# dayne-2stacks/Fingerprint-Matching-Code

Measured on AMD Instinct MI355X. Metric: graph-match pairs/sec @ n=256 kpts, batch=1024, 1 & 8 GPU, higher is better.
Workload: dtype bf16

## Files before the change

### fingerprint-matching-code_amd/_lib.py

```python
import ctypes
import os

_HERE = os.path.dirname(os.path.abspath(__file__))
LIB_PATH = os.environ.get("FPM_LIB_PATH") or os.path.join(_HERE, "libfpm_hip.so")

P = ctypes.c_void_p
I = ctypes.c_int
L = ctypes.c_long
F = ctypes.c_float

SIGNATURES = {
    "fpm_last_error": (ctypes.c_char_p, []),
    "fpm_version": (I, []),
    "fpm_device_sync": (I, []),
    "fpm_sinkhorn_log_fwd": (I, [P, L, L, L, P, L, L, L, P, P, I, I, I, I, F, I, P]),
    "fpm_sinkhorn_ws_bytes": (L, [I, I, I]),
    "fpm_sinkhorn_log_fwd_ws": (I, [P, L, L, L, P, L, L, L, P, P, I, I, I, I, F, I, P, L, P]),
    "fpm_soft_topk_fwd": (I, [P, L, L, P, P, P, I, I, I, I, F, P, L, L, P, P, L, L, P]),
    "fpm_topk_select": (I, [P, L, L, P, L, P, I, I, I, P, L, L, P, L, L, P]),
    "fpm_greedy_perm": (I, [P, L, I, P, I, I, I, P, L, L, P]),
    "fpm_gemm": (I, [I, P, L, L, P, P, L, L, I, I, I, I, I, P, P, P, L, L, P, P, P]),
    "fpm_cast_bf16": (I, [P, P, L, P]),
    "fpm_global_weights": (I, [P, L, P, L, I, I, I, P, L, P]),
    "fpm_coef_tanh": (I, [P, L, P, P, I, I, I, P, L, P]),
    "fpm_split_bf16x3": (I, [P, L, L, I, I, P, L, P]),
    "fpm_set_tuning": (I, [ctypes.c_char_p, I]),
    "fpm_spline_plan_bytes": (L, [L, L]),
    "fpm_spline_plan": (I, [P, P, P, L, L, I, P, L, P]),
    "fpm_spline_plan_graphs": (I, [P, P, P, L, L, I, L, P, L, P]),
    "fpm_spline_plan_csr": (I, [P, L, L, ctypes.POINTER(P), ctypes.POINTER(P)]),
    "fpm_spline_plan_edges": (I, [P, L, L, ctypes.POINTER(P), ctypes.POINTER(P), ctypes.POINTER(P)]),
    "fpm_spline_plan_multi": (I, [P, I, I, I, P, P]),
    "fpm_spline_plan_job_bytes": (I, []),
    "fpm_spline_y_bytes": (L, [I, L, L]),
    "fpm_spline_conv_fwd": (I, [I, P, P, L, L, I, P, P, P, P, L, I, P, P, P, P, P]),
    "fpm_spline_conv_fwd_argmax": (I, [I, P, P, L, L, I, P, P, P, P, L, I, P, P, P, P, P, P]),
    "fpm_edge_diff": (I, [P, P, P, L, I, P, P]),
    "fpm_rows_bcast_scale": (I, [I, P, L, I, P, P, P, I, P]),
    "fpm_rows_gather_scale": (I, [I, P, P, P, I, I, I, P, P, P, I, P]),
    "fpm_rank_topk": (I, [P, L, I, I, I, P, P, P]),
    "fpm_rank_select_ws_bytes": (L, [I]),
    "fpm_rank_select": (I, [P, L, I, I, I, P, P, P, L, P]),
    "fpm_group_scores": (I, [P, L, I, I, P, L, P, L, I, I, P, P, P]),
    "fpm_coarse_score_wide_ws_bytes": (L, [I]),
    "fpm_coarse_score_stream_ws_bytes": (L, [I, I, I]),
    "fpm_rows_fetch": (I, [P, L, P, P, I, I, I, P, L, P, P]),
    "fpm_rows_pack": (I, [P, L, P, I, I, P, P, P, L, P]),
    "fpm_edge_diff_padded":(I, [P, P, P, P, P, P, L, I, P, P]),
    "fpm_kron_gnn_layer_fwd": (I, [P, I, I, I, I, P, P, P, P, P, P, P, P, P, P, P, P]),
    "fpm_kron_gnn_layer_fwd_ord": (I, [P, I, I, I, I, P, P, P, P, P, P, P, P, P, P, P, P, P]),
    "fpm_gnn_param_count": (I, [I]),
    "fpm_node_classifier": (I, [P, I, I, I, P, P, P, P, P]),
    "fpm_crossset_attn_fwd": (I, [I, P, L, L, I, I, I, P, P, I, P, P, P, P, P, P, P]),
    "fpm_instnorm": (I, [I, P, P, I, I, I, P, P, P, P, F, P, P, I, P, P]),
    "fpm_afau_head": (I, [P, P, I, I, P, P, P, P, P, P, P, P, P, P]),
    "fpm_afau_head_bwd": (I, [P, P, I, I, P, P, P, P, P, P, P, P, P, P, P, P, P]),
    "fpm_instnorm_bwd": (I, [P, P, I, I, I, P, P, P, P, F, P, P, P, I, P, P, P]),
    "fpm_afau_attn_bwd": (I, [P, L, L, I, I, I, P, P, I, P, P, P, P, P, P, P, P, P, P]),
    "fpm_rows_sum": (I, [P, I, L, P, I, P, I, P]),
    "fpm_transpose": (I, [P, L, I, L, P, L, P]),
    "fpm_elementwise": (I, [P, P, L, I, P]),
    "fpm_outer_sum_parts": (L, [I, L]),
    "fpm_outer_sum": (I, [P, L, L, I, P, L, L, I, I, I, L, P, P]),
    "fpm_bn_ws_floats": (L, [I, I]),
    "fpm_bn_relu_train_fwd": (I, [P, I, I, L, P, P, F, F, P, P, P, P, P, P]),
    "fpm_bn_relu_train_bwd": (I, [P, P, I, I, L, P, P, P, P, P, P, P]),
    "fpm_match_cls_ws_floats": (L, [I, I, I]),
    "fpm_match_cls_fwd": (I, [I, P, P, I, I, I, P, P, P, P, P, P, P, P, P, P, P, P, P, P]),
    "fpm_match_cls_train_ws_floats": (L, [I, I, I, I]),
    "fpm_match_cls_train_fwd": (I, [P, P, I, I, I] + [P] * 14 + [ctypes.c_float, ctypes.c_float, P, P, P, P]),
    "fpm_match_cls_train_bwd": (I, [P, P, I, I, I] + [P] * 21 + [P]),
    "fpm_gemm_norm_max": (I, [P, L, P, L, I, I, I, P, P, L, P, P, ctypes.c_float, I, P, P]),
    "fpm_gemm_norm_out": (I, [P, L, P, L, I, I, I, P, P, P, ctypes.c_float, I, P, L, P, L, P]),
    "fpm_affinity_ws_floats": (L, [I, I, I]),
    "fpm_perm_loss_fwd": (I, [P, L, L, P, L, L, P, P, I, I, I, P, P, P, P]),
    "fpm_perm_loss_bwd": (I, [P, L, L, P, L, L, P, P, I, I, I, P, P, P, P]),
    "fpm_affinity_fwd": (I, [P, L, P, L, P, I, P, P, I, I, I, I, P, P, I, P, L, P, L, P]),
    "fpm_gemm_x3out": (I, [P, L, P, L, I, I, I, I, P, P, P, ctypes.c_float, I, P, L, P, L, I, P]),
    "fpm_lsa_batch_host": (I, [P, L, L, P, P, I, I, P, I]),
    "fpm_lsa_submit": (L, [P, L, L, P, P, I, I, P, I]),
    "fpm_lsa_wait": (I, [L, I, ctypes.POINTER(ctypes.c_double)]),
    "fpm_lsa_batch_device": (I, [P, L, L, P, P, I, I, I, P, P, P]),
    "fpm_csr_dot_csc_to_dense": (I, [I, P, P, P, P, P, P, L, L, L, P, P]),
    "fpm_dense_dot_csc_to_dense": (I, [I, P, P, P, P, L, L, L, L, P, P]),
    "fpm_csr_dot_diag_to_csr": (I, [I, P, P, P, P, L, L, L, P, P]),
    "fpm_bilinear_diag": (I, [I, P, P, P, P, L, P, P, P, L, L, P, P]),
    "fpm_csr_dot_csc_to_csr_host": (L, [I, P, P, P, P, P, P, L, L, L, P, L, P, P]),
    "fpm_csr_dot_diag_to_csr_host": (I, [I, P, P, P, P, L, L, L, P]),
    "fpm_bilinear_diag_host": (I, [I, P, P, P, P, L, P, P, P, L, L, P]),
    "fpm_gconv_ws_floats": (L, [I, I, I]),
    "fpm_gconv_fwd": (I, [P, P, I, I, I, I, P, P, I, P, P, P]),
    "fpm_graph_words": (I, [I]),
    "fpm_graph_build": (I, [P, P, I, I, I, ctypes.c_double, P, P, P, P, P]),
    "fpm_graph_edges": (I, [P, P, P, P, I, I, ctypes.c_double, P, P, P, P, P, P, I, P]),
    "fpm_kron_pattern": (I, [P, P, L, P, P, L, I, I, I, I, P, P, P]),
    "fpm_feature_align_ws_floats": (L, [P, P]),
    "fpm_feature_align_fwd": (I, [P, P, P, P, P, P, P, P, I, F, F, P, P, L, P, P]),
    "fpm_feature_align_bwd": (I, [P, P, P, P, P, P, P, P, I, F, F, P, P, L, P, P, P, P, P, P]),
    "fpm_sinkhorn_bwd_ws_floats": (L, [I, I, I, I]),
    "fpm_sinkhorn_log_bwd": (I, [P, L, L, L, P, L, L, L, P, P, P, I, I, I, I, F, I, P, L, P]),
    "fpm_soft_topk_bwd_ws_floats": (L, [I, I, I]),
    "fpm_soft_topk_bwd": (I, [P, L, L, P, P, P, P, I, I, I, F, P, L, L, P, P, L, P, P]),
    "fpm_spline_plan_rows": (I, [P, L, L, ctypes.POINTER(P), ctypes.POINTER(P)]),
    "fpm_spline_conv_bwd_data": (I, [I, P, L, L, I, P, P, P, I, P, P, P, P, P, P, I, P]),
# ... 56 lines not shown
```

### fingerprint-matching-code_amd/csrc/gemm.hip

```cpp
#include "gemm_phase.h"
#include <cstdlib>
#include <cstring>

namespace fpm {
int& gemm_bn256_min();
}
int& gemm_store_sc1_flag();

extern "C" int fpm_gemm(int dtype, const void* A, long lda, long sA, const int* a_rows, const void* B, long ldb,
                        long sB, int M, int N, int K, int batch, int epi, const float* bias, float* Cf, void* Ct,
                        long ldc, long sC, const int* n1, const int* n2, void* stream) {
    using namespace fpm;
    FPM_CHECK_ARG(dtype == 0 || dtype == 1, "gemm: dtype must be 0 (f32) or 1 (bf16)");
    FPM_CHECK_ARG(M >= 0 && N > 0 && K > 0 && batch >= 0, "gemm: bad sizes M=%d N=%d K=%d", M, N, K);
    FPM_CHECK_ARG(K % (dtype ? 8 : 4) == 0, "gemm: K=%d must be a multiple of %d", K, dtype ? 8 : 4);
    FPM_CHECK_ARG(lda % (dtype ? 8 : 4) == 0 && ldb % (dtype ? 8 : 4) == 0, "gemm: lda/ldb must keep rows 16-B aligned");
    FPM_CHECK_ARG((epi != EPI_AFFINITY && epi != EPI_HALF_AFFINITY) || (n1 && n2),
                  "gemm: affinity epilogues need n1/n2");
    FPM_CHECK_ARG(epi >= EPI_STORE && epi <= EPI_HALF_AFFINITY, "gemm: bad epilogue %d", epi);
    if (M == 0 || batch == 0) return 0;
    GemmParams p = {};
    p.A = A; p.lda = lda; p.sA = sA; p.a_rows = a_rows;
    p.B = B; p.ldb = ldb; p.sB = sB; p.sB_seg = 0;
    p.row_scale = nullptr;
// ... 154 lines not shown
    else hipLaunchKernelGGL((gemm_big_kernel<128, EPI_STORE, true>), grid, dim3(G2_THREADS), 0, st, p);
    return check_launch("fpm_gemm_x3out");
}

namespace {
__global__ __launch_bounds__(256) void rows_scale_kernel(const float* __restrict__ X, long ldx, int nmax, int d,
                                                         const float* __restrict__ coef, float* __restrict__ Xc) {
    const long r = blockIdx.x;
    const int b = (int)(r / nmax);
    for (int k = threadIdx.x; k < d; k += 256) Xc[r * d + k] = X[r * ldx + k] * coef[(long)b * d + k];
}
}

extern "C" long fpm_affinity_ws_floats(int B, int n1max, int d) { return (long)B * d + (long)B * n1max * d; }

extern "C" int fpm_affinity_fwd(const float* X1, long ld1, const float* X2, long ld2, const float* w, int kw,
                                const float* A_w, const float* A_b, int B, int n1max, int n2max, int d, const int* n1,
                                const int* n2, int epi, float* K, long ldk, float* ws, long ws_floats, void* stream) {
    using namespace fpm;
    FPM_CHECK_ARG(epi == 0 || epi == 1, "affinity_fwd: epi must be 0 (vertex) or 1 (edge)");
    FPM_CHECK_ARG(B >= 0 && n1max > 0 && n2max > 0 && d > 0 && d % 4 == 0 && kw > 0 && kw % 4 == 0,
                  "affinity_fwd: bad sizes");
    FPM_CHECK_ARG(ld1 >= d && ld2 >= d && ld2 % 4 == 0 && ldk >= n2max, "affinity_fwd: bad strides");
    FPM_CHECK_ARG(ws && ws_floats >= fpm_affinity_ws_floats(B, n1max, d), "affinity_fwd: workspace too small");
    FPM_CHECK_ARG(n1 && n2 && K && X1 && X2 && w && A_w, "affinity_fwd: null operand");
    if (B == 0) return 0;
    float* coef = ws;
    float* X1c = ws + (long)B * d;
    if (fpm_gemm(0, w, kw, 0, nullptr, A_w, kw, 0, B, d, kw, 1, EPI_TANH, A_b, coef, nullptr, d, 0, nullptr, nullptr,
                 stream))
        return 1;
    hipLaunchKernelGGL(rows_scale_kernel, dim3((unsigned)((long)B * n1max)), dim3(256), 0, (hipStream_t)stream, X1,
                       ld1, n1max, d, coef, X1c);
    if (check_launch("fpm_affinity_fwd")) return 1;
    return fpm_gemm(0, X1c, d, (long)n1max * d, nullptr, X2, ld2, (long)n2max * ld2, n1max, n2max, d, B,
                    epi == 0 ? EPI_AFFINITY : EPI_HALF_AFFINITY, nullptr, K, nullptr, ldk, (long)n1max * ldk, n2, n1,
                    stream);
}

int& plan_graph_flag();
int& combine_npb_flag();
int& sinkhorn_bwd_reg_flag();
int& sinkhorn_fast_flag();
int& sinkhorn_lform_flag();
int& soft_topk_fast_flag();
int& afau_attn_v_flag();
int& gnn_store_sc1_flag();
int& combine_store_sc1_flag();
int& gemm_store_sc1_flag();
int& combine_lds_kb_flag();
int& gnn_mlp_off_flag();
int& outer_sum_vec_flag();
int& gnn_sweeps_flag();
int& scatter_f32_rows_flag();
int& scatter_batch_flag();
int& afau_head_split_flag();

extern "C" int fpm_set_tuning(const char* key, int value) {
    int* f = nullptr;
    if (key && !strcmp(key, "gemm_phase")) f = &fpm::gemm_phase_flag();
    else if (key && !strcmp(key, "gemm_walk")) f = &fpm::gemm_walk_flag();
    else if (key && !strcmp(key, "gemm_bn256_min")) f = &fpm::gemm_bn256_min();
    else if (key && !strcmp(key, "plan_graph")) f = &plan_graph_flag();
    else if (key && !strcmp(key, "combine_npb")) f = &combine_npb_flag();
    else if (key && !strcmp(key, "sinkhorn_bwd_reg")) f = &sinkhorn_bwd_reg_flag();
    else if (key && !strcmp(key, "sinkhorn_fast")) f = &sinkhorn_fast_flag();
    else if (key && !strcmp(key, "sinkhorn_lform")) f = &sinkhorn_lform_flag();
    else if (key && !strcmp(key, "topk_fast")) f = &soft_topk_fast_flag();
    else if (key && !strcmp(key, "afau_attn_v")) f = &afau_attn_v_flag();
    else if (key && !strcmp(key, "gnn_store_sc1")) f = &gnn_store_sc1_flag();
    else if (key && !strcmp(key, "combine_store_sc1")) f = &combine_store_sc1_flag();
    else if (key && !strcmp(key, "gemm_store_sc1")) f = &gemm_store_sc1_flag();
    else if (key && !strcmp(key, "combine_lds_kb")) f = &combine_lds_kb_flag();
    else if (key && !strcmp(key, "gnn_mlp_off")) f = &gnn_mlp_off_flag();
    else if (key && !strcmp(key, "outer_sum_vec")) f = &outer_sum_vec_flag();
    else if (key && !strcmp(key, "gnn_sweeps")) f = &gnn_sweeps_flag();
    else if (key && !strcmp(key, "scatter_f32_rows")) f = &scatter_f32_rows_flag();
    else if (key && !strcmp(key, "scatter_batch")) f = &scatter_batch_flag();
    else if (key && !strcmp(key, "afau_head_split")) f = &afau_head_split_flag();
    if (!f) {
        fpm::set_error("fpm_set_tuning: unknown key '%s'", key ? key : "(null)");
        return -1;
    }
    if (f == &gnn_mlp_off_flag() && value != 0) {
        const char* e = getenv("FPM_TIMING_PROBES");
        if (!e || strcmp(e, "1") != 0) {
            fpm::set_error("fpm_set_tuning: '%s' is a timing probe with wrong results; set FPM_TIMING_PROBES=1 "
                           "to allow it", key);
            return -1;
        }
    }
    const int prev = *f;
    *f = value;
    return prev;
}

namespace {
__global__ void cast_bf16_kernel(const float* __restrict__ x, bf16_t* __restrict__ y, long n) {
    long i = (long)blockIdx.x * blockDim.x + threadIdx.x;
    long stride = (long)gridDim.x * blockDim.x;
    for (; i < n; i += stride) y[i] = fpm::f2bf(x[i]);
}

__global__ __launch_bounds__(256) void cast_bf16_v8_kernel(const float4* __restrict__ x, uint4* __restrict__ y, long n8) {
    const long i = (long)blockIdx.x * blockDim.x + threadIdx.x;
    if (i >= n8) return;
    const float4 a = x[2 * i], b = x[2 * i + 1];
    uint4 o;
    o.x = (uint32_t)fpm::f2bf(a.x) | ((uint32_t)fpm::f2bf(a.y) << 16);
    o.y = (uint32_t)fpm::f2bf(a.z) | ((uint32_t)fpm::f2bf(a.w) << 16);
    o.z = (uint32_t)fpm::f2bf(b.x) | ((uint32_t)fpm::f2bf(b.y) << 16);
    o.w = (uint32_t)fpm::f2bf(b.z) | ((uint32_t)fpm::f2bf(b.w) << 16);
    y[i] = o;
}
}

extern "C" int fpm_cast_bf16(const float* x, void* y, long n, void* stream) {
    if (n <= 0) return 0;
    if (n % 8 == 0 && ((uintptr_t)x & 15) == 0 && ((uintptr_t)y & 15) == 0) {
        const long n8 = n / 8;
        hipLaunchKernelGGL(cast_bf16_v8_kernel, dim3((unsigned)((n8 + 255) / 256)), dim3(256), 0, (hipStream_t)stream,
                           (const float4*)x, (uint4*)y, n8);
        return fpm::check_launch("fpm_cast_bf16");
    }
    long blocks = (n + 255) / 256;
    if (blocks > 65536) blocks = 65536;
    hipLaunchKernelGGL(cast_bf16_kernel, dim3(blocks), dim3(256), 0, (hipStream_t)stream, x, (bf16_t*)y, n);
    return fpm::check_launch("fpm_cast_bf16");
}
// ... 122 lines not shown
```

### fingerprint-matching-code_amd/csrc/gnn.hip

```cpp
#include "fpm_common.h"
#include <cstdlib>

namespace {

__device__ __forceinline__ bool pair_block(int n2max, int B, int& b, int& d) {
    const int x = blockIdx.x & 7, k = blockIdx.x >> 3;
    b = (k / n2max) * 8 + x;
    d = k % n2max;
    return b < B;
}

inline unsigned pair_grid(int n2max, int B) { return (unsigned)(((B + 7) / 8) * 8 * n2max); }

template <int C>
struct GnnPack {
    static constexpr int Wl = 0, bl = Wl + 16 * C, Wr = bl + 16, W1 = Wr + 16 * C, b1 = W1 + 16 * C, W2 = b1 + 16,
                         b2 = W2 + 256, wc = b2 + 16, bc = wc + 16, total = bc + 1;
};

typedef float f2_t __attribute__((ext_vector_type(2)));

__device__ __forceinline__ void pk_fma_bcast(f2_t& acc, f2_t w, f2_t v, bool hi) {
    if (hi) asm("v_pk_fma_f32 %0, %1, %2, %0 op_sel:[0,1,0] op_sel_hi:[1,1,1]" : "+v"(acc) : "s"(w), "v"(v));
    else asm("v_pk_fma_f32 %0, %1, %2, %0 op_sel_hi:[1,0,1]" : "+v"(acc) : "s"(w), "v"(v));
}

template <int C, int TS, int SPOL = 0, bool MLP = true>
__device__ __forceinline__ void gnn_point(const float* Tg, __amdgpu_buffer_rsrc_t xr, int N4, long N, int n1max,
                                          int b, int d, int i, int nn2, const int* __restrict__ ptr1,
                                          const int* __restrict__ nbr1, int n1b, int n2b, const float* __restrict__ W,
                                          float* __restrict__ Xo, float* __restrict__ zbuf, float* __restrict__ vpart,
                                          const float* __restrict__ cls_w) {
    using P = GnnPack<C>;
    const long p = (long)d * n1max + i;
    const __amdgpu_buffer_rsrc_t orr = __builtin_amdgcn_make_buffer_rsrc((void*)(Xo + (long)b * 17 * N), (short)0,
                                                                         (int)(17 * N * 4), 0x00020000);
    auto store_o = [&](int o, float v) {
        __builtin_amdgcn_raw_buffer_store_b32(__float_as_uint(v), orr, (int)p * 4, o * N4, SPOL);
    };
    const int beg = ptr1[(long)b * n1max + i], end = ptr1[(long)b * n1max + i + 1];
    const bool self = p < (long)n1b * n2b;
    float x[C], agg[C];
#pragma unroll
    for (int c = 0; c < C; ++c) {
        x[c] = __uint_as_float(__builtin_amdgcn_raw_buffer_load_b32(xr, (int)p * 4, c * N4, 0));
        agg[c] = 0.f;
    }
    for (int e = beg; e < end; ++e) {
        const float* Ta = Tg + nbr1[e] * TS;
        if constexpr (C == 17) {
            static_assert(TS % 4 == 0, "16-B aligned node rows");
#pragma unroll
            for (int q = 0; q < 4; ++q) {
// ... 110 lines not shown
                load_row(nbr2[k], va);
#pragma unroll
                for (int c = 0; c < C; ++c) acc[c] += va[c];
            }
        } else {
            constexpr int GS = (C + NSW - 1) / NSW;
#pragma unroll
            for (int g0 = 0; g0 < C; g0 += GS) {
                int k = beg2;
                for (; k + 3 < end2; k += 4) {
                    float v[4][GS];
#pragma unroll
                    for (int u = 0; u < 4; ++u) {
                        const int r = nbr2[k + u];
#pragma unroll
                        for (int c = 0; c < GS; ++c)
                            if (g0 + c < C)
                                v[u][c] = __uint_as_float(__builtin_amdgcn_raw_buffer_load_b32(xr, (r * n1max + i) * 4,
                                                                                                (g0 + c) * N4, 0));
                    }
#pragma unroll
                    for (int u = 0; u < 4; ++u)
#pragma unroll
                        for (int c = 0; c < GS; ++c)
                            if (g0 + c < C) acc[g0 + c] += v[u][c];
                }
                for (; k < end2; ++k) {
                    const int r = nbr2[k];
#pragma unroll
                    for (int c = 0; c < GS; ++c)
                        if (g0 + c < C)
                            acc[g0 + c] += __uint_as_float(__builtin_amdgcn_raw_buffer_load_b32(xr, (r * n1max + i) * 4,
                                                                                                 (g0 + c) * N4, 0));
                }
            }
        }
        float* Ti = T + i * TS;
        if constexpr (C == 17) {
#pragma unroll
            for (int q = 0; q < 4; ++q)
                *(float4*)(Ti + 4 * q) = make_float4(acc[4 * q], acc[4 * q + 1], acc[4 * q + 2], acc[4 * q + 3]);
            Ti[16] = acc[16];
        } else {
            Ti[0] = acc[0];
        }
    }
    __syncthreads();
    if (i >= n1max) return;
    gnn_point<C, TS, SPOL, MLP>(T, xr, N4, N, n1max, b, d, i, end2 - beg2, ptr1, nbr1, n1[b], n2[b], W, Xo, zbuf,
                                vpart, cls_w);
    (void)NSW;
}

__global__ __launch_bounds__(256) void node_classifier_t_kernel(const float* __restrict__ X, int n1max, int n2max,
                                                                const float* __restrict__ w,
                                                                const float* __restrict__ bias,
                                                                const float* __restrict__ vpart,
                                                                float* __restrict__ s) {
    __shared__ float tile[64][65];
    const int b = blockIdx.z, d0 = blockIdx.y * 64, i0 = blockIdx.x * 64;
    const int tx = threadIdx.x & 63, ty = threadIdx.x >> 6;
    const long N = (long)n1max * n2max;
    const float* Xb = X + (long)b * 17 * N;
    const int i = i0 + tx;
#pragma unroll 4
    for (int r = 0; r < 16; ++r) {
        const int d = d0 + ty + 4 * r;
        if (d < n2max && i < n1max) {
            const long p = (long)d * n1max + i;
            float acc;
            if (vpart) {
                acc = fmaf(w[16], Xb[16L * N + p], vpart[(long)b * N + p]);
            } else {
                acc = 0.f;
#pragma unroll
                for (int c = 0; c < 17; ++c) acc += w[c] * Xb[(long)c * N + p];
            }
            tile[tx][ty + 4 * r] = acc + bias[0];
        }
    }
    __syncthreads();
    const int d = d0 + tx;
#pragma unroll 4
    for (int r = 0; r < 16; ++r) {
        const int ii = i0 + ty + 4 * r;
        if (ii < n1max && d < n2max) s[(long)b * N + (long)ii * n2max + d] = tile[ty + 4 * r][tx];
    }
}

}

int& gnn_sweeps_flag() {
    static int v = [] {
        const char* e = getenv("FPM_GNN_SWEEPS");
        return e ? atoi(e) : 1;
    }();
    return v;
}

int& gnn_store_sc1_flag() {
    static int v = [] {
        const char* e = getenv("FPM_GNN_SC1");
        return e ? atoi(e) : 0;
    }();
    return v;
}

int& gnn_mlp_off_flag() {
    static int v = 0;
    return v;
}

extern "C" int fpm_kron_gnn_layer_fwd_ord(const float* X, int C, int B, int n1max, int n2max, const int* ptr1,
                                          const int* nbr1, const int* ptr2, const int* nbr2, const int* n1,
                                          const int* n2, const float* params, float* Xout, float* zbuf,
                                          float* vpart, const float* cls_w, const int* ord2, void* stream) {
    FPM_CHECK_ARG(C == 1 || C == 17, "gnn_layer: C must be 1 or 17 (got %d)", C);
    FPM_CHECK_ARG(!vpart || cls_w, "gnn_layer: vpart needs cls_w");
    if (B == 0) return 0;
    FPM_CHECK_ARG(n1max >= 1 && n1max <= 1024, "gnn_layer: n1max must be in [1, 1024]");
    FPM_CHECK_ARG((long)17 * n1max * n2max * 4 < (1L << 31), "gnn_layer: a pair's state must be < 2 GiB");
    const size_t sh = (size_t)(C == 1 ? 1 : 20) * n1max * 4;
    const int threads = (n1max + 63) / 64 * 64;
    void (*k)(const float*, int, int, const int*, const int*, const int*, const int*, const int*, const int*,
              const float*, float*, float*, float*, const float*, int, const int*) =
        (C == 17 && gnn_sweeps_flag() == 2 && !gnn_mlp_off_flag() && !gnn_store_sc1_flag()) ? gnn_layer_kernel<17, 0, true, 2>
        : (C == 17 && gnn_sweeps_flag() == 3 && !gnn_mlp_off_flag() && !gnn_store_sc1_flag()) ? gnn_layer_kernel<17, 0, true, 3>
        : gnn_mlp_off_flag() ? (C == 1 ? gnn_layer_kernel<1, 0, false> : gnn_layer_kernel<17, 0, false>)
        : gnn_store_sc1_flag() ? (C == 1 ? gnn_layer_kernel<1, 16> : gnn_layer_kernel<17, 16>)
                               : (C == 1 ? gnn_layer_kernel<1> : gnn_layer_kernel<17>);
    if (sh > 65536) (void)hipFuncSetAttribute((const void*)k, hipFuncAttributeMaxDynamicSharedMemorySize, (int)sh);
    hipLaunchKernelGGL(k, dim3(pair_grid(n2max, B)), dim3(threads), sh, (hipStream_t)stream, X, n1max, n2max, ptr1,
                       nbr1, ptr2, nbr2, n1, n2, params, Xout, zbuf, vpart, cls_w, B, ord2);
    return fpm::check_launch("fpm_kron_gnn_layer_fwd");
}

extern "C" int fpm_kron_gnn_layer_fwd(const float* X, int C, int B, int n1max, int n2max, const int* ptr1,
                                      const int* nbr1, const int* ptr2, const int* nbr2, const int* n1,
                                      const int* n2, const float* params, float* Xout, float* zbuf,
                                      float* vpart, const float* cls_w, void* stream) {
    return fpm_kron_gnn_layer_fwd_ord(X, C, B, n1max, n2max, ptr1, nbr1, ptr2, nbr2, n1, n2, params, Xout, zbuf,
                                      vpart, cls_w, nullptr, stream);
}

extern "C" int fpm_gnn_param_count(int C) { return C == 1 ? GnnPack<1>::total : GnnPack<17>::total; }

extern "C" int fpm_node_classifier(const float* X, int B, int n1max, int n2max, const float* w, const float* bias,
                                   const float* vpart, float* s, void* stream) {
    if (B == 0) return 0;
    FPM_CHECK_ARG(B <= 65535, "node_classifier: B must be <= 65535");
    const dim3 grid((unsigned)((n1max + 63) / 64), (unsigned)((n2max + 63) / 64), (unsigned)B);
    hipLaunchKernelGGL(node_classifier_t_kernel, grid, dim3(256), 0, (hipStream_t)stream, X, n1max, n2max, w, bias,
                       vpart, s);
    return fpm::check_launch("fpm_node_classifier");
}

namespace {
__global__ __launch_bounds__(1024) void kron_agg_kernel(const float* __restrict__ X, int C, int n1max, int n2max,
                                                        const int* __restrict__ tptr1, const int* __restrict__ tnbr1,
                                                        const int* __restrict__ tptr2, const int* __restrict__ tnbr2,
                                                        const int* __restrict__ q1, const int* __restrict__ q2,
                                                        const int* __restrict__ n1, const int* __restrict__ n2,
                                                        int adj_flags, float* __restrict__ out, int B) {
    extern __shared__ float T[];
    int d, b;
    if (!pair_block(n2max, B, b, d)) return;
    const int adj = adj_flags & 1;
    const bool accum = (adj_flags & 2) != 0;
    const int i = threadIdx.x;
    const long N = (long)n1max * n2max;
    const float* Xb = X + (long)b * C * N;
    const long nb1 = (long)b * n1max, nb2 = (long)b * n2max;
    const long nn = (long)n1[b] * n2[b];
    auto den = [&](int dd, int ii) -> float {
        const int g1 = q1[nb1 + ii + 1] - q1[nb1 + ii];
        const int g2 = q2[nb2 + dd + 1] - q2[nb2 + dd];
        return (float)(g1 * g2 + (((long)dd * n1max + ii) < nn ? 1 : 0));
    };
    auto xval = [&](int c, int dd, int ii) -> float {
        const float x = Xb[(long)c * N + (long)dd * n1max + ii];
        if (!adj) return x;
        const float dn = den(dd, ii);
        return dn > 0.f ? x / dn : 0.f;
// ... 205 lines not shown
```

### fingerprint-matching-code_amd/ops.py

```python
import ctypes

import torch

from . import _lib

F32, BF16 = 0, 1
EPI_STORE, EPI_RELU, EPI_TANH, EPI_AFFINITY, EPI_HALF_AFFINITY = 0, 1, 2, 3, 4
EPI_NORM_OUT = 6


def _p(t):
    return ctypes.c_void_p(0 if t is None else t.data_ptr())


def _stream(t=None):
    dev = t.device if t is not None else torch.device("cuda")
    return ctypes.c_void_p(torch.cuda.current_stream(dev).cuda_stream)


def _dev(*ts):
    for t in ts:
        if t is not None and not t.is_cuda:
            raise _lib.FpmError("fpm op called with a CPU tensor: the HIP path has no CPU fallback")

# ... 780 lines not shown
            raise _lib.FpmError("%s: qidx value outside [0, %d)" % (op, Q))
        ng, nq = oh[gh + 1] - oh[gh], qoh[qh + 1] - qoh[qh]
        nqmax, ngmax = int(nq.max()), int(ng.max())
        for what, n in (("probe", nq), ("selected entry", ng)):
            if int(n.max()) > nmax or int(n.min()) < 1:
                raise _lib.FpmError("%s: a %s of %d keypoints; the %s coarse pass takes 1 to %s = %d"
                                    % (op, what, int(n.max()) if int(n.max()) > nmax else int(n.min()), kernel, bound,
                                       nmax))
    iters, tau = _check_iters_tau(op, iters, tau)
    if not y.is_cuda:
        dtype = _host_dtype(op, dtype)
        res = torch.empty(B, dtype=dtype)
        for b in range(B):
            q = int(qh[b])
            res[b:b + 1] = _coarse_score_host(y, oh, gh[b:b + 1], yq[int(qoh[q]):int(qoh[q + 1])], coef[b:b + 1], iters,
                                              tau, dtype)
        return _coarse_out(op, y, B, out, dtype, res)
    out = _coarse_out(op, y, B, out, dtype)
    if B:
        _coarse_call(kernel, True, y, (_p(y), _p(row_off), _p(gidx), G, B, _p(yq), _p(qrow_off), _p(qidx), Q, _p(coef),
                                       iters, tau, _p(out)), B, nqmax, ngmax)
    return out


def edge_diff(x, src, dst):
    _dev(x, src, dst)
    E, D = src.numel(), x.shape[-1]
    out = torch.empty(E, D, device=x.device, dtype=torch.float32)
    _lib.call("fpm_edge_diff", _p(x), _p(src), _p(dst), E, D, _p(out), _stream(x))
    return out


def edge_diff_padded(x, src, dst, pair, row, nrows, cscale=None):
    _dev(x, src, dst, pair, row)
    E, D = src.numel(), x.shape[-1]
    out = torch.zeros(nrows, D, device=x.device, dtype=torch.float32)
    _lib.call("fpm_edge_diff_padded", _p(x), _p(src), _p(dst), _p(pair), _p(row), _p(cscale), E, D, _p(out),
              _stream(x))
    return out


def gnn_layer(X, C, B, n1max, n2max, csr1, csr2, n1, n2, params, Xout, zbuf, vpart=None, cls_w=None, ord2=None):
    _dev(X, n1, n2, params, Xout, zbuf, vpart, cls_w, ord2)
    _shape(X, (B, C, n2max, n1max), "gnn_layer X")
    _shape(Xout, (B, 17, n2max, n1max), "gnn_layer Xout")
    _shape(zbuf, (B, n2max, n1max), "gnn_layer zbuf")
    _shape(vpart, (B, n2max, n1max), "gnn_layer vpart")
    _shape(ord2, (B, n2max), "gnn_layer ord2")
    _lib.call("fpm_kron_gnn_layer_fwd_ord", _p(X), C, B, n1max, n2max, ctypes.c_void_p(csr1[0]),
              ctypes.c_void_p(csr1[1]), ctypes.c_void_p(csr2[0]), ctypes.c_void_p(csr2[1]), _p(n1), _p(n2),
              _p(params), _p(Xout), _p(zbuf), _p(vpart), _p(cls_w), _p(ord2), _stream(X))


def node_classifier(X, B, n1max, n2max, w, b, out, vpart=None):
    _dev(X, w, b, out, vpart)
    _shape(X, (B, 17, n2max, n1max), "node_classifier X")
    _shape(out, (B, n1max, n2max), "node_classifier out")
    _shape(vpart, (B, n2max, n1max), "node_classifier vpart")
    _lib.call("fpm_node_classifier", _p(X), B, n1max, n2max, _p(w), _p(b), _p(vpart), _p(out), _stream(X))


def crossset_attn(cost, n2, Wv, mix1w, mix1b, mix2w, mix2b, out, split=False, stats=None):
    _dev(cost, n2, Wv, out)
    B, n1max, n2max = cost.shape
    _shape(out, (B * n1max, 768 if split else 256), "crossset_attn out")
    if split and out.dtype != torch.bfloat16:
        raise _lib.FpmError("crossset_attn: split rows are bf16")
    _shape(stats, (B * n1max, 16, 2), "crossset_attn stats")
    if n2max > 1 and cost.stride(2) != 1:
        raise _lib.FpmError("crossset_attn: cost rows must be contiguous (inner stride %d)" % cost.stride(2))
    _lib.call("fpm_crossset_attn_fwd", 2 if split else _code(out), _p(cost), cost.stride(0), cost.stride(1), B, n1max, n2max,
              _p(n2), _p(Wv), Wv.shape[1], _p(mix1w), _p(mix1b), _p(mix2w), _p(mix2b), _p(out), _p(stats),
              _stream(cost))


def instnorm(in1, B, P, Cn, w, b, in2=None, nvalid=None, onehot_bias=None, out_f=None, out_t=None, gmax=None,
             eps=1e-5, ldt=0):
    code = _code(out_t) if out_t is not None else F32
    ref = in1 if in1 is not None else w
    _lib.call("fpm_instnorm", code, _p(in1), _p(in2), B, P, Cn, _p(nvalid), _p(onehot_bias), _p(w), _p(b),
              float(eps), _p(out_f), _p(out_t), int(ldt), _p(gmax), _stream(ref))


def gemm_norm_max(A, Bw, M, N, K, lda, ldb, bias, res, nw, nb, gmax, P=256, eps=1e-5):
    _dev(A, Bw, res, gmax)
    _lib.call("fpm_gemm_norm_max", _p(A), int(lda), _p(Bw), int(ldb), int(M), int(N), int(K), _p(bias), _p(res),
              int(res.stride(0)), _p(nw), _p(nb), float(eps), int(P), _p(gmax), _stream(A))
    return gmax


def gemm_norm_out(A, Bw, M, N, K, lda, ldb, bias, nw, nb, out_f, out_t=None, ldt=0, P=256, eps=1e-5):
    _dev(A, Bw, out_f)
    _lib.call("fpm_gemm_norm_out", _p(A), int(lda), _p(Bw), int(ldb), int(M), int(N), int(K), _p(bias), _p(nw),
              _p(nb), float(eps), int(P), _p(out_f), int(out_f.stride(0)), _p(out_t),
              int(ldt or (out_t.stride(0) if out_t is not None else 0)), _stream(A))
    return out_f


def affinity(X1, X2, w, A_w, A_b, n1, n2, half=False, out=None):
    _dev(X1, X2, w, A_w, A_b, n1, n2)
    for t in (X1, X2, w, A_w, A_b):
        if t.dtype != torch.float32:
            raise _lib.FpmError("affinity: float32 operands expected")
    B, n1max, d = X1.shape
    n2max = X2.shape[1]
    kw = w.shape[1]
# ... 537 lines not shown
```

### include/fpm.h

```cpp
#ifndef FPM_H_
#define FPM_H_

#ifdef __cplusplus
extern "C" {
#endif

const char* fpm_last_error(void);
int fpm_version(void);
int fpm_device_sync(void);

int fpm_sinkhorn_log_fwd(const float* s, long s_sb, long s_si, long s_sj, float* out, long o_sb, long o_si,
                         long o_sj, const int* n1, const int* n2, int B, int n1max, int n2max, int iters,
                         float tau, int dummy_row, void* stream);
long fpm_sinkhorn_ws_bytes(int B, int n1max, int n2max);
int fpm_sinkhorn_log_fwd_ws(const float* s, long s_sb, long s_si, long s_sj, float* out, long o_sb, long o_si,
                            long o_sj, const int* n1, const int* n2, int B, int n1max, int n2max, int iters,
                            float tau, int dummy_row, void* ws, long ws_bytes, void* stream);

int fpm_soft_topk_fwd(const float* ss, long s_sb, long s_ld, const int* n1, const int* n2, const float* k, int B,
                      int n1max, int n2max, int iters, float tau, float* out, long o_sb, long o_ld, int* steps_out,
                      float* out2, long o2_sb, long o2_ld, void* stream);

int fpm_topk_select(const float* ds, long d_sb, long d_ld, const int* assign, long a_sb, const float* k, int B,
                    int n1max, int n2max, float* perm, long p_sb, long p_ld, float* lsa_out, long l_sb, long l_ld,
// ... 21 lines not shown
                  long ldo, void* stream);
long fpm_affinity_ws_floats(int B, int n1max, int d);
int fpm_affinity_fwd(const float* X1, long ld1, const float* X2, long ld2, const float* w, int kw, const float* A_w,
                     const float* A_b, int B, int n1max, int n2max, int d, const int* n1, const int* n2, int epi,
                     float* K, long ldk, float* ws, long ws_floats, void* stream);

int fpm_perm_loss_fwd(const float* ds, long d_sb, long d_ld, const float* gt, long g_sb, long g_ld, const int* n1,
                      const int* n2, int B, int n1max, int n2max, float* ws, int* bad, float* out, void* stream);
int fpm_perm_loss_bwd(const float* ds, long d_sb, long d_ld, const float* gt, long g_sb, long g_ld, const int* n1,
                      const int* n2, int B, int n1max, int n2max, const float* g, float* ws, float* dds, void* stream);

int fpm_gemm_x3out(const void* A, long lda, const void* B, long ldb, int M, int N, int K, int epi, const float* bias,
                   const float* nw, const float* nb, float eps, int P, float* out_f, long ldc, void* out_t3, long ldt,
                   int Kp, void* stream);
int fpm_set_tuning(const char* key, int value);

long fpm_spline_plan_bytes(long E, long num_nodes);
long fpm_spline_y_bytes(int dtype, long E, long num_nodes);
int fpm_spline_plan(const int* src, const int* dst, const float* pseudo, long E, long num_nodes, int nmax, void* ws,
                    long ws_bytes, void* stream);
int fpm_spline_plan_graphs(const int* src, const int* dst, const float* pseudo, long E, long num_nodes, int nmax,
                           long max_graph_edges, void* ws, long ws_bytes, void* stream);
int fpm_spline_plan_csr(void* ws, long E, long num_nodes, int** dst_ptr, int** nbr_local);
int fpm_spline_plan_edges(void* ws, long E, long num_nodes, int** csr_e, int** rows4, float** basis4);
int fpm_spline_plan_multi(const void* jobs, int njobs, int total_graphs, int nmax, void* ws, void* stream);
int fpm_spline_plan_job_bytes(void);
int fpm_spline_conv_fwd(int dtype, const void* x_op, const void* plan_ws, long E, long num_nodes, int nmax,
                        const int* nvalid, const void* W, const float* bias, void* y_ws, long y_ws_bytes, int mode,
                        const float* xres, const float* cscale, float* out_f, void* out_t, void* stream);
int fpm_spline_conv_fwd_argmax(int dtype, const void* x_op, const void* plan_ws, long E, long num_nodes, int nmax,
                               const int* nvalid, const void* W, const float* bias, void* y_ws, long y_ws_bytes,
                               int mode, const float* xres, const float* cscale, float* out_f, void* out_t,
                               int* argmax, void* stream);
int fpm_rows_bcast_scale(int dtype, const float* y, long rows, int B, const float* coef, float* out_f, void* out_t,
                         int split, void* stream);
int fpm_rows_gather_scale(int dtype, const float* y, const long* row_off, const int* idx, int G, int B, int nmax,
                          const float* coef, float* out_f, void* out_t, int split, void* stream);
int fpm_rows_fetch(const float* src, long src_rows, const long* row_off, const int* idx, int G, int M, int nmax,
                   float* out, long out_rows, const long* out_off, void* stream);
int fpm_rows_pack(const float* src, long src_rows, const int* n, int B, int nmax, const long* out_off, float* out32,
                  void* out16, long out_rows, void* stream);
int fpm_edge_diff(const float* x, const int* src, const int* dst, long E, int D, float* out, void* stream);
int fpm_edge_diff_padded(const float* x, const int* src, const int* dst, const int* pair, const int* row,
                         const float* cscale, long E, int D, float* out, void* stream);

int fpm_kron_gnn_layer_fwd(const float* X, int C, int B, int n1max, int n2max, const int* ptr1, const int* nbr1,
                           const int* ptr2, const int* nbr2, const int* n1, const int* n2, const float* params,
                           float* Xout, float* zbuf, float* vpart, const float* cls_w, void* stream);
int fpm_kron_gnn_layer_fwd_ord(const float* X, int C, int B, int n1max, int n2max, const int* ptr1,
                               const int* nbr1, const int* ptr2, const int* nbr2, const int* n1, const int* n2,
                               const float* params, float* Xout, float* zbuf, float* vpart, const float* cls_w,
                               const int* ord2, void* stream);
int fpm_gnn_param_count(int C);
int fpm_node_classifier(const float* X, int B, int n1max, int n2max, const float* w, const float* bias,
                        const float* vpart, float* s, void* stream);

int fpm_crossset_attn_fwd(int dtype, const float* cost, long c_sb, long c_ld, int B, int n1max, int n2max,
                          const int* n2, const float* Wv, int emb, const float* mix1w, const float* mix1b,
                          const float* mix2w, const float* mix2b, void* out, float* stats, void* stream);
int fpm_instnorm(int dtype, const float* in1, const float* in2, int B, int P, int Cn, const int* nvalid,
                 const float* onehot_bias, const float* w, const float* bias, float eps, float* out_f, void* out_t,
                 int ldt, float* gmax, void* stream);
int fpm_afau_head(const float* gr, const float* gc, int B, int E, const float* r0w, const float* r0b,
                  const float* r2w, const float* r2b, const float* c0w, const float* c0b, const float* c2w,
                  const float* c2b, float* ks, void* stream);

int fpm_kron_gnn_layer_fwd_f64(const void* X, int x_f64, int C, int B, int n1max, int n2max, const int* ptr1,
                               const int* nbr1, const int* ptr2, const int* nbr2, const int* n1, const int* n2,
                               const float* params, double* Xout, double* zbuf, void* stream);
int fpm_sinkhorn_log_fwd_f64(const void* s, int s_f64, long s_sb, long s_si, long s_sj, double* o64, long o_sb,
                             long o_si, long o_sj, float* o32, long f_sb, long f_si, long f_sj, const int* n1,
                             const int* n2, int B, int n1max, int n2max, int iters, double tau, int dummy_row,
                             void* stream);
int fpm_node_classifier_f64(const double* X, int B, int n1max, int n2max, const float* w, const float* bias,
                            double* s64, float* s32, void* stream);
int fpm_crossset_attn_row_f64(const double* cost, long c_sb, long c_ld, int B, int n1max, int n2max, const int* n2,
                              const double* Wv, int emb, const double* mix1w, const double* mix1b,
                              const double* mix2w, const double* mix2b, double* out, void* stream);
int fpm_gemm_f64(const double* A, int lda, const double* W, int ldw, const double* bias, double* C, int ldc, int M,
                 int N, int K, int relu, void* stream);
int fpm_instnorm_f64(const double* in1, const double* in2, int B, int P, int Cn, const int* nvalid,
                     const double* onehot_bias, const double* w, const double* bias, double eps, double* out,
                     double* gmax, void* stream);
int fpm_afau_head_f64(const double* gr, const double* gc, const int* cidx, int B, int E, const double* r0w,
                      const double* r0b, const double* r2w, const double* r2b, const double* c0w, const double* c0b,
                      const double* c2w, const double* c2b, float* ks, void* stream);
int fpm_soft_topk_fwd_f64(const double* ss, long s_sb, long s_ld, const int* n1, const int* n2, const float* k, int B,
                          int n1max, int n2max, int iters, double tau, double* ws, long ws_doubles, float* out,
                          long o_sb, long o_ld, int* steps_out, float* out2, long o2_sb, long o2_ld, void* stream);

int fpm_afau_head_bwd(const float* gr, const float* gc, int B, int E, const float* r0w, const float* r0b,
                      const float* r2w, const float* r2b, const float* c0w, const float* c0b, const float* c2w,
                      const float* c2b, const float* dks, float* dgr, float* dgc, float* part, void* stream);
int fpm_instnorm_bwd(const float* in1, const float* in2, int B, int P, int Cn, const int* nvalid,
                     const float* onehot_bias, const float* w, const float* bias, float eps, const float* dy,
                     const float* gseed, float* dx, int accumulate, float* dw_part, float* db_part, void* stream);
int fpm_afau_attn_bwd(const float* cost, long c_sb, long c_ld, int B, int n1max, int n2max, const int* n2,
                      const float* Wv, int emb, const float* mix1w, const float* mix1b, const float* mix2w,
                      const float* mix2b, const float* att_out, const float* datt, const float* stats,
                      float* dwv_part, float* mix_part, void* stream);
int fpm_rows_sum(const float* in, int B, long K, const int* key, int nkeys, float* out, int accumulate,
                 void* stream);
int fpm_transpose(const float* in, long R, int C, long ldi, float* out, long ldo, void* stream);
int fpm_elementwise(float* x, const float* ref, long n, int mode, void* stream);

long fpm_outer_sum_parts(int B, long N);
// ... 165 lines not shown
```

Measured before the change: 32100.

## Add LDS-resident GNN layer kernel with reduced shared memory and higher occupancy

Adds a new Kronecker GNN layer kernel that aggregates the second-graph neighbours per pair into a compact LDS table (18 floats per node instead of 20), then gathers first-graph neighbours through hand-written ds_read_b64 loads and buffer loads. It is launched with launch bounds requesting 8 waves per SIMD, and becomes the default when n1max is at most 256 and the default sweep and MLP settings are active. The aim is to cut LDS footprint and register pressure so more blocks stay resident, and to speed up the gather loop. The inline asm forces a full lgkmcnt wait after each pair of reads, which limits overlap. An occupancy query entry point is also exposed.

```diff
diff --git a/fingerprint-matching-code_amd/_lib.py b/fingerprint-matching-code_amd/_lib.py
--- a/fingerprint-matching-code_amd/_lib.py
+++ b/fingerprint-matching-code_amd/_lib.py
@@ -50,6 +50,7 @@
     "fpm_kron_gnn_layer_fwd": (I, [P, I, I, I, I, P, P, P, P, P, P, P, P, P, P, P, P]),
     "fpm_kron_gnn_layer_fwd_ord": (I, [P, I, I, I, I, P, P, P, P, P, P, P, P, P, P, P, P, P]),
     "fpm_gnn_param_count": (I, [I]),
+    "fpm_gnn_resident_blocks": (I, [I, I]),
     "fpm_node_classifier": (I, [P, I, I, I, P, P, P, P, P]),
     "fpm_crossset_attn_fwd": (I, [I, P, L, L, I, I, I, P, P, I, P, P, P, P, P, P, P]),
     "fpm_instnorm": (I, [I, P, P, I, I, I, P, P, P, P, F, P, P, I, P, P]),
diff --git a/fingerprint-matching-code_amd/csrc/gemm.hip b/fingerprint-matching-code_amd/csrc/gemm.hip
--- a/fingerprint-matching-code_amd/csrc/gemm.hip
+++ b/fingerprint-matching-code_amd/csrc/gemm.hip
@@ -230,6 +230,7 @@
 int& gnn_mlp_off_flag();
 int& outer_sum_vec_flag();
 int& gnn_sweeps_flag();
+int& gnn_form_flag();
 int& scatter_f32_rows_flag();
 int& scatter_batch_flag();
 int& afau_head_split_flag();
@@ -253,6 +254,7 @@
     else if (key && !strcmp(key, "gnn_mlp_off")) f = &gnn_mlp_off_flag();
     else if (key && !strcmp(key, "outer_sum_vec")) f = &outer_sum_vec_flag();
     else if (key && !strcmp(key, "gnn_sweeps")) f = &gnn_sweeps_flag();
+    else if (key && !strcmp(key, "gnn_form")) f = &gnn_form_flag();
     else if (key && !strcmp(key, "scatter_f32_rows")) f = &scatter_f32_rows_flag();
     else if (key && !strcmp(key, "scatter_batch")) f = &scatter_batch_flag();
     else if (key && !strcmp(key, "afau_head_split")) f = &afau_head_split_flag();
diff --git a/fingerprint-matching-code_amd/csrc/gnn.hip b/fingerprint-matching-code_amd/csrc/gnn.hip
--- a/fingerprint-matching-code_amd/csrc/gnn.hip
+++ b/fingerprint-matching-code_amd/csrc/gnn.hip
@@ -1,4 +1,5 @@
 #include "fpm_common.h"
+#include <cstdint>
 #include <cstdlib>
 
 namespace {
@@ -215,6 +216,172 @@
     (void)NSW;
 }
 
+template <int C>
+__device__ __forceinline__ void gnn_resident_body(float* T, const float* __restrict__ X, int n1max, int n2max,
+                                                  const int* __restrict__ ptr1, const int* __restrict__ nbr1,
+                                                  const int* __restrict__ ptr2, const int* __restrict__ nbr2,
+                                                  const int* __restrict__ n1, const int* __restrict__ n2,
+                                                  const float* __restrict__ W, float* __restrict__ Xo,
+                                                  float* __restrict__ zbuf, float* __restrict__ vpart,
+                                                  const float* __restrict__ cls_w, int B,
+                                                  const int* __restrict__ ord2) {
+    using P = GnnPack<C>;
+    constexpr int CP = (C + 1) / 2;
+    constexpr int TS = C == 1 ? 1 : 2 * CP;
+    int b, d;
+    if (!pair_block(n2max, B, b, d)) return;
+    if (ord2) d = ord2[(long)b * n2max + d];
+    const int i = threadIdx.x;
+    const long N = (long)n1max * n2max;
+    const __amdgpu_buffer_rsrc_t xr =
+        __builtin_amdgcn_make_buffer_rsrc((void*)(X + (long)b * C * N), (short)0, (int)(C * N * 4), 0x00020000);
+    const int N4 = (int)(N * 4);
+    const int beg2 = ptr2[(long)b * n2max + d], end2 = ptr2[(long)b * n2max + d + 1];
+    auto load_row = [&](int off, f2_t (&v)[CP]) {
+#pragma unroll
+        for (int k = 0; k < CP; ++k) {
+            v[k].x = __uint_as_float(__builtin_amdgcn_raw_buffer_load_b32(xr, off, 2 * k * N4, 0));
+            v[k].y = 2 * k + 1 < C ? __uint_as_float(__builtin_amdgcn_raw_buffer_load_b32(xr, off, (2 * k + 1) * N4, 0))
+                                   : 0.f;
+        }
+    };
+    if (i < n1max) {
+        f2_t acc[CP];
+#pragma unroll
+        for (int k = 0; k < CP; ++k) acc[k] = (f2_t){0.f, 0.f};
+        int k = beg2;
+        for (; k + 1 < end2; k += 2) {
+            f2_t va[CP], vb[CP];
+            load_row((nbr2[k] * n1max + i) * 4, va);
+            load_row((nbr2[k + 1] * n1max + i) * 4, vb);
+#pragma unroll
+            for (int q = 0; q < CP; ++q) acc[q] += va[q];
+#pragma unroll
+            for (int q = 0; q < CP; ++q) acc[q] += vb[q];
+        }
+        if (k < end2) {
+            f2_t va[CP];
+            load_row((nbr2[k] * n1max + i) * 4, va);
+#pragma unroll
+            for (int q = 0; q < CP; ++q) acc[q] += va[q];
+        }
+        float* Ti = T + i * TS;
+        if constexpr (C == 1) {
+            Ti[0] = acc[0].x;
+        } else {
+#pragma unroll
+            for (int q = 0; q < CP; ++q) *(f2_t*)(Ti + 2 * q) = acc[q];
+        }
+    }
+    __syncthreads();
+    if (i >= n1max) return;
+
+    const int nn2 = end2 - beg2;
+    const int p4 = (d * n1max + i) * 4;
+    const __amdgpu_buffer_rsrc_t orr = __builtin_amdgcn_make_buffer_rsrc((void*)(Xo + (long)b * 17 * N), (short)0,
+                                                                         (int)(17 * N * 4), 0x00020000);
+    const f2_t* W2p = (const f2_t*)W;
+    f2_t x2[CP];
+    load_row(p4, x2);
+    f2_t u[8];
+    {
+        f2_t h[8];
+#pragma unroll
+        for (int m = 0; m < 8; ++m) {
+            f2_t s = W2p[(P::b1 >> 1) + m];
+#pragma unroll
+            for (int c = 0; c < C; ++c) pk_fma_bcast(s, W2p[((P::W1 + c * 16) >> 1) + m], x2[c >> 1], c & 1);
+            h[m] = (f2_t){fmaxf(s.x, 0.f), fmaxf(s.y, 0.f)};
+        }
+#pragma unroll
+        for (int op = 0; op < 8; ++op) {
+            f2_t t = {0.f, 0.f};
+#pragma unroll
+            for (int m = 0; m < 16; ++m) pk_fma_bcast(t, W2p[((P::W2 + m * 16) >> 1) + op], h[m >> 1], m & 1);
+            const f2_t tb = t + W2p[(P::b2 >> 1) + op];
+            u[op] = (f2_t){fmaxf(tb.x, 0.f), fmaxf(tb.y, 0.f)};
+        }
+    }
+    const int base1 = ptr1[(long)b * n1max];
+    const __amdgpu_buffer_rsrc_t nr =
+        __builtin_amdgcn_make_buffer_rsrc((void*)(nbr1 + base1), (short)0, 0x7ffffffc, 0x00020000);
+    const int beg = ptr1[(long)b * n1max + i] - base1, end = ptr1[(long)b * n1max + i + 1] - base1;
+    f2_t a2[CP];
+#pragma unroll
+    for (int q = 0; q < CP; ++q) a2[q] = (f2_t){0.f, 0.f};
+    const unsigned tbase = (unsigned)(uintptr_t)(__attribute__((address_space(3))) float*)T;
+    for (int e4 = beg * 4; e4 < end * 4; e4 += 4) {
+        const int a = __builtin_amdgcn_raw_buffer_load_b32(nr, e4, 0, 0);
+        if constexpr (C == 1) {
+            a2[0].x += T[a];
+        } else {
+            const unsigned ta = tbase + a * (TS * 4);
+#define FPM_GNN_READ2(q0, o0, o1)                                                                                \
+    {                                                                                                            \
+        f2_t g0, g1;                                                                                             \
+        asm volatile("ds_read_b64 %0, %2 offset:" #o0 "\n\tds_read_b64 %1, %2 offset:" #o1                       \
+                     "\n\ts_waitcnt lgkmcnt(0)"                                                                  \
+                     : "=&v"(g0), "=&v"(g1)                                                                      \
+                     : "v"(ta)                                                                                   \
+                     : "memory");                                                                                \
+        a2[q0] += g0;                                                                                            \
+        a2[q0 + 1] += g1;                                                                                        \
+    }
+            FPM_GNN_READ2(0, 0, 8)
+            FPM_GNN_READ2(2, 16, 24)
+            FPM_GNN_READ2(4, 32, 40)
+            FPM_GNN_READ2(6, 48, 56)
+#undef FPM_GNN_READ2
+            {
+                f2_t g0;
+                asm volatile("ds_read_b64 %0, %1 offset:64\n\ts_waitcnt lgkmcnt(0)" : "=&v"(g0) : "v"(ta) : "memory");
+                a2[8] += g0;
+            }
+        }
+    }
+    const bool self = (p4 >> 2) < n1[b] * n2[b];
+    const float cnt = (float)((end - beg) * nn2 + (self ? 1 : 0));
+    const float rc = cnt > 0.f ? 1.f / cnt : 0.f;
+#pragma unroll
+    for (int q = 0; q < CP; ++q) {
+        const f2_t v = self ? a2[q] + x2[q] : a2[q];
+        a2[q] = v * rc;
+    }
+    float z = 0.f, vp = 0.f;
+#pragma unroll
+    for (int op = 0; op < 8; ++op) {
+        const int o = 2 * op;
+        f2_t l = {0.f, 0.f}, r = {0.f, 0.f};
+#pragma unroll
+        for (int c = 0; c < C; ++c) {
+            pk_fma_bcast(l, W2p[((P::Wl + c * 16) >> 1) + op], a2[c >> 1], c & 1);
+            pk_fma_bcast(r, W2p[((P::Wr + c * 16) >> 1) + op], x2[c >> 1], c & 1);
+        }
+        const f2_t x1 = ((l + W2p[(P::bl >> 1) + op]) + r) + u[op];
+        if (vpart) {
+            vp = fmaf(cls_w[o], x1.x, vp);
+            vp = fmaf(cls_w[o + 1], x1.y, vp);
+        } else {
+            __builtin_amdgcn_raw_buffer_store_b32(__float_as_uint(x1.x), orr, p4, o * N4, 0);
+            __builtin_amdgcn_raw_buffer_store_b32(__float_as_uint(x1.y), orr, p4, (o + 1) * N4, 0);
+        }
+        z = fmaf(W[P::wc + o], x1.x, z);
+        z = fmaf(W[P::wc + o + 1], x1.y, z);
+    }
+    if (vpart) vpart[(long)b * N + (p4 >> 2)] = vp;
+    zbuf[(long)b * N + (p4 >> 2)] = z + W[P::bc];
+}
+
+template <int C, int WPS>
+__global__ __launch_bounds__(256, WPS) void gnn_layer_resident_kernel(
+    const float* __restrict__ X, int n1max, int n2max, const int* __restrict__ ptr1, const int* __restrict__ nbr1,
+    const int* __restrict__ ptr2, const int* __restrict__ nbr2, const int* __restrict__ n1, const int* __restrict__ n2,
+    const float* __restrict__ W, float* __restrict__ Xo, float* __restrict__ zbuf, float* __restrict__ vpart,
+    const float* __restrict__ cls_w, int B, const int* __restrict__ ord2) {
+    extern __shared__ __attribute__((aligned(16))) float T[];
+    gnn_resident_body<C>(T, X, n1max, n2max, ptr1, nbr1, ptr2, nbr2, n1, n2, W, Xo, zbuf, vpart, cls_w, B, ord2);
+}
+
 __global__ __launch_bounds__(256) void node_classifier_t_kernel(const float* __restrict__ X, int n1max, int n2max,
                                                                 const float* __restrict__ w,
                                                                 const float* __restrict__ bias,
@@ -274,6 +441,46 @@
     return v;
 }
 
+int& gnn_form_flag() {
+    static int v = [] {
+        const char* e = getenv("FPM_GNN_FORM");
+        return e ? atoi(e) : 1;
+    }();
+    return v;
+}
+
+namespace {
+typedef void (*gnn_kernel_t)(const float*, int, int, const int*, const int*, const int*, const int*, const int*,
+                             const int*, const float*, float*, float*, float*, const float*, int, const int*);
+
+bool gnn_resident(int n1max) {
+    return gnn_form_flag() != 0 && n1max <= 256 && gnn_sweeps_flag() == 1 && !gnn_mlp_off_flag() &&
+           !gnn_store_sc1_flag();
+}
+
+gnn_kernel_t gnn_resident_kernel(int C) {
+    return C == 1 ? gnn_layer_resident_kernel<1, 8> : gnn_layer_resident_kernel<17, 8>;
+}
+
+size_t gnn_resident_lds(int C, int n1max) { return (size_t)(C == 1 ? 1 : 18) * n1max * 4; }
+}
+
+extern "C" int fpm_gnn_resident_blocks(int C, int n1max) {
+    FPM_CHECK_ARG(C == 1 || C == 17, "gnn_resident_blocks: C must be 1 or 17 (got %d)", C);
+    FPM_CHECK_ARG(n1max >= 1 && n1max <= 1024, "gnn_resident_blocks: n1max must be in [1, 1024]");
+    const bool res = gnn_resident(n1max);
+    const gnn_kernel_t k = res ? gnn_resident_kernel(C)
+                               : (C == 1 ? gnn_layer_kernel<1> : gnn_layer_kernel<17>);
+    const size_t sh = res ? gnn_resident_lds(C, n1max) : (size_t)(C == 1 ? 1 : 20) * n1max * 4;
+    if (sh > 65536) (void)hipFuncSetAttribute((const void*)k, hipFuncAttributeMaxDynamicSharedMemorySize, (int)sh);
+    int nb = 0;
+    if (hipOccupancyMaxActiveBlocksPerMultiprocessor(&nb, (const void*)k, (n1max + 63) / 64 * 64, sh) != hipSuccess) {
+        fpm::set_error("gnn_resident_blocks: the occupancy query failed");
+        return -1;
+    }
+    return nb;
+}
+
 extern "C" int fpm_kron_gnn_layer_fwd_ord(const float* X, int C, int B, int n1max, int n2max, const int* ptr1,
                                           const int* nbr1, const int* ptr2, const int* nbr2, const int* n1,
                                           const int* n2, const float* params, float* Xout, float* zbuf,
@@ -283,15 +490,18 @@
     if (B == 0) return 0;
     FPM_CHECK_ARG(n1max >= 1 && n1max <= 1024, "gnn_layer: n1max must be in [1, 1024]");
     FPM_CHECK_ARG((long)17 * n1max * n2max * 4 < (1L << 31), "gnn_layer: a pair's state must be < 2 GiB");
-    const size_t sh = (size_t)(C == 1 ? 1 : 20) * n1max * 4;
+    size_t sh = (size_t)(C == 1 ? 1 : 20) * n1max * 4;
     const int threads = (n1max + 63) / 64 * 64;
-    void (*k)(const float*, int, int, const int*, const int*, const int*, const int*, const int*, const int*,
-              const float*, float*, float*, float*, const float*, int, const int*) =
+    gnn_kernel_t k =
         (C == 17 && gnn_sweeps_flag() == 2 && !gnn_mlp_off_flag() && !gnn_store_sc1_flag()) ? gnn_layer_kernel<17, 0, true, 2>
         : (C == 17 && gnn_sweeps_flag() == 3 && !gnn_mlp_off_flag() && !gnn_store_sc1_flag()) ? gnn_layer_kernel<17, 0, true, 3>
         : gnn_mlp_off_flag() ? (C == 1 ? gnn_layer_kernel<1, 0, false> : gnn_layer_kernel<17, 0, false>)
         : gnn_store_sc1_flag() ? (C == 1 ? gnn_layer_kernel<1, 16> : gnn_layer_kernel<17, 16>)
                                : (C == 1 ? gnn_layer_kernel<1> : gnn_layer_kernel<17>);
+    if (gnn_resident(n1max)) {
+        k = gnn_resident_kernel(C);
+        sh = gnn_resident_lds(C, n1max);
+    }
     if (sh > 65536) (void)hipFuncSetAttribute((const void*)k, hipFuncAttributeMaxDynamicSharedMemorySize, (int)sh);
     hipLaunchKernelGGL(k, dim3(pair_grid(n2max, B)), dim3(threads), sh, (hipStream_t)stream, X, n1max, n2max, ptr1,
                        nbr1, ptr2, nbr2, n1, n2, params, Xout, zbuf, vpart, cls_w, B, ord2);
diff --git a/fingerprint-matching-code_amd/ops.py b/fingerprint-matching-code_amd/ops.py
--- a/fingerprint-matching-code_amd/ops.py
+++ b/fingerprint-matching-code_amd/ops.py
@@ -856,6 +856,13 @@
               _p(params), _p(Xout), _p(zbuf), _p(vpart), _p(cls_w), _p(ord2), _stream(X))
 
 
+def gnn_resident_blocks(C, n1max):
+    nb = int(_lib.load().fpm_gnn_resident_blocks(int(C), int(n1max)))
+    if nb < 0:
+        raise _lib.FpmError(_lib.load().fpm_last_error().decode(errors="replace"))
+    return nb
+
+
 def node_classifier(X, B, n1max, n2max, w, b, out, vpart=None):
     _dev(X, w, b, out, vpart)
     _shape(X, (B, 17, n2max, n1max), "node_classifier X")
diff --git a/include/fpm.h b/include/fpm.h
--- a/include/fpm.h
+++ b/include/fpm.h
@@ -97,6 +97,7 @@
                                const float* params, float* Xout, float* zbuf, float* vpart, const float* cls_w,
                                const int* ord2, void* stream);
 int fpm_gnn_param_count(int C);
+int fpm_gnn_resident_blocks(int C, int n1max);
 int fpm_node_classifier(const float* X, int B, int n1max, int n2max, const float* w, const float* bias,
                         const float* vpart, float* s, void* stream);
 
```

New measurement: 32530, median of 6. 1.01x the previous value.
